# mgtools/DCTdomain

Hardware: AMD Instinct MI355X
Metric: DCT fingerprints/sec on L=500 D=1280 (higher is better)
Workload: dtype f64

## Files before the change

### dctdomain_amd/csrc/dctfp.hip

```cpp
#include "dctfp.h"

#include <hip/hip_runtime.h>

#include <dlfcn.h>
#include <execinfo.h>
#include <signal.h>
#include <unistd.h>

#include <algorithm>
#include <cmath>
#include <cstdarg>
#include <cstdio>
#include <cstring>
#include <map>
#include <mutex>
#include <new>
#include <string>
#include <unordered_map>
#include <vector>

#include "launch.h"
#include "reccut_kernel.hip.h"

using namespace dctfp;
// ... 1808 lines not shown
    return DCTFP_OK;
} DCTFP_GUARD("dctfp_scale")

int dctfp_gather_rows(dctfp_ctx* ctx, const void* embed, int32_t dtype, int64_t n_rows, int64_t n_cols, int64_t ld,
                      const dctfp_piece* pieces, int64_t n_pieces, double* out, void* stream_v) try {
    if (!ctx || !embed || !pieces || !out) return fail(DCTFP_ERR_INVALID, "dctfp_gather_rows: NULL argument");
    std::lock_guard<std::mutex> lock(ctx->mu);
    if (dtype != DCTFP_F32 && dtype != DCTFP_F64) return fail(DCTFP_ERR_INVALID, "dctfp_gather_rows: dtype %d", dtype);
    if (n_pieces < 1 || n_pieces > 65535 || n_cols < 1 || ld < n_cols) return fail(DCTFP_ERR_INVALID, "dctfp_gather_rows: bad shape");
    hipStream_t stream = (hipStream_t)stream_v;
    HIP_TRY(hipSetDevice(ctx->device));
    const size_t esz = dtype == DCTFP_F32 ? 4 : 8;
    TableLease tables(ctx->ring, stream);
    int rc = tables.stage((size_t)n_pieces * sizeof(PieceA));
    if (rc) return rc;
    PieceA* h = (PieceA*)tables.host();
    uint64_t t0 = 0;
    uint32_t max_rows = 0;
    for (int64_t i = 0; i < n_pieces; ++i) {
        const dctfp_piece& pc = pieces[i];
        if (pc.n_rows <= 0 || pc.row_start < 0 || pc.row_start + pc.n_rows > n_rows)
            return fail(DCTFP_ERR_INVALID, "dctfp_gather_rows: piece %lld outside the matrix", (long long)i);
        h[i].ptr = (const char*)embed + (size_t)pc.row_start * (size_t)ld * esz;
        h[i].n_rows = (uint32_t)pc.n_rows;
        h[i].t0 = (uint32_t)t0;
        t0 += (uint64_t)pc.n_rows;
        max_rows = std::max(max_rows, (uint32_t)pc.n_rows);
        if (t0 > 0x7fffffffu) return fail(DCTFP_ERR_LIMIT, "dctfp_gather_rows: more than 2^31 rows");
    }
    rc = tables.upload((size_t)n_pieces * sizeof(PieceA), stream);
    if (rc) return rc;
    const unsigned gx = (unsigned)std::min<int64_t>(((int64_t)max_rows * n_cols + 255) / 256, 2048);
    if (dtype == DCTFP_F32)
        hipLaunchKernelGGL((gather_rows_kernel<float>), dim3(gx, (unsigned)n_pieces), dim3(256), 0, stream, (const PieceA*)tables.dev(), (int)n_pieces, n_cols, ld, out);
    else
        hipLaunchKernelGGL((gather_rows_kernel<double>), dim3(gx, (unsigned)n_pieces), dim3(256), 0, stream, (const PieceA*)tables.dev(), (int)n_pieces, n_cols, ld, out);
    HIP_TRY(hipGetLastError());
    return tables.release();
} DCTFP_GUARD("dctfp_gather_rows")


int dctfp_contact_topk(dctfp_ctx* ctx, const void* const* maps, const int64_t* ld, const int32_t* n_res,
                       int32_t n_prot, double t, int32_t* out_i, int32_t* out_j, float* out_v,
                       const int64_t* out_offs, int32_t* out_n, void* stream_v) try {
    if (!ctx || !maps || !ld || !n_res || !out_i || !out_j || !out_v || !out_offs || !out_n)
        return fail(DCTFP_ERR_INVALID, "dctfp_contact_topk: NULL argument");
    std::lock_guard<std::mutex> lock(ctx->mu);
    if (n_prot < 0) return fail(DCTFP_ERR_INVALID, "dctfp_contact_topk: negative count");
    if (n_prot == 0) return DCTFP_OK;
    hipStream_t stream = (hipStream_t)stream_v;
    HIP_TRY(hipSetDevice(ctx->device));
    const int64_t kLongPairs = (int64_t)1 << 18;
    constexpr int64_t kStripePairs = (int64_t)1 << 17;
    auto is_long = [&](int64_t L, int64_t cand) {
        const int64_t k = dctfp_contact_count((int32_t)L, t);
        return k > 0 && (cand >= kLongPairs || (k > 3000 && cand >= ((int64_t)1 << 19)));
    };
    std::vector<int32_t> order((size_t)n_prot);
    int32_t n_short = 0, n_long = 0;
    int64_t n_stripes = 0;
    for (int32_t p = 0; p < n_prot; ++p) {
        const int64_t L = n_res[p];
        if (L < 0 || (L > 0 && (!maps[p] || ld[p] < L)))
            return fail(DCTFP_ERR_INVALID, "dctfp_contact_topk: protein %d: bad map", p);
        const int64_t cand = L >= 6 ? (L - 5) * (L - 4) / 2 : 0;
        if (is_long(L, cand)) {
            ++n_long;
            n_stripes += std::min<int64_t>(512, (cand + kStripePairs - 1) / kStripePairs);
        } else {
            ++n_short;
        }
    }
    {
        int32_t a = 0, b = n_short;
        for (int32_t p = 0; p < n_prot; ++p) {
            const int64_t L = n_res[p];
            const int64_t cand = L >= 6 ? (L - 5) * (L - 4) / 2 : 0;
            if (is_long(L, cand)) order[b++] = p;
            else order[a++] = p;
        }
    }
    const size_t off_stripe = align_up((size_t)n_prot * sizeof(TopkJob), 16);
    const size_t off_first = align_up(off_stripe + (size_t)n_stripes * sizeof(TopkStripe), 16);
    const size_t off_state = align_up(off_first + (size_t)n_long * sizeof(int32_t), 16);
    const size_t up_bytes = align_up(off_state + (size_t)n_long * sizeof(TopkState), 16);
    const size_t off_ties = up_bytes;
    const size_t all_bytes = off_ties + (size_t)n_stripes * sizeof(int32_t);
    TableLease tables(ctx->ring, stream);
    Fork fork(stream);
    int rc = tables.stage(up_bytes);
    if (rc) return rc;
    TopkJob* h = (TopkJob*)tables.host();
    TopkStripe* hs = (TopkStripe*)(tables.host() + off_stripe);
    int32_t* hfirst = (int32_t*)(tables.host() + off_first);
    TopkState* hstate = (TopkState*)(tables.host() + off_state);
    int64_t s_fill = 0;
    for (int32_t q = 0; q < n_prot; ++q) {
        const int32_t p = order[q];
        const int64_t L = n_res[p];
        h[q].map = (const float*)maps[p];
        h[q].ld = ld[p];
        h[q].n_res = (int32_t)L;
        h[q].k = (int32_t)dctfp_contact_count((int32_t)L, t);
        h[q].out_off = out_offs[p];
        h[q].orig = p;
        h[q].reserved = 0;
        if (out_offs[p + 1] - out_offs[p] < h[q].k)
            return fail(DCTFP_ERR_INVALID, "dctfp_contact_topk: protein %d: output room %lld < %d", p,
                        (long long)(out_offs[p + 1] - out_offs[p]), h[q].k);
        if (q >= n_short) {
            const int32_t lj = q - n_short;
            const int64_t cand = (L - 5) * (L - 4) / 2;
            const int64_t ns = std::min<int64_t>(512, (cand + kStripePairs - 1) / kStripePairs);
            hfirst[lj] = (int32_t)s_fill;
            memset(&hstate[lj], 0, sizeof(TopkState));
            hstate[lj].need = h[q].k;
            int64_t acc = 0;
            int32_t row = 0, stripe = 0;
            const int32_t last_row = (int32_t)L - 5;
            for (int64_t k = 0; k < ns; ++k) {
                const int64_t goal = cand * (k + 1) / ns;
                const int32_t begin = row;
                while (row < last_row && (acc < goal || k + 1 == ns)) {
                    acc += L - 5 - row;
                    ++row;
                }
                if (row > begin) {
                    TopkStripe& sp = hs[s_fill++];
                    sp.job = lj;
                    sp.row_begin = begin;
                    sp.row_end = row;
                    sp.stripe = stripe++;
                }
            }
        }
    }
    const int64_t used_stripes = s_fill;
    rc = tables.upload(up_bytes, stream, all_bytes);
    if (rc) return rc;
    const TopkJob* djobs = (const TopkJob*)tables.dev();
    const bool long_beside = n_long > 0 && used_stripes > 0 && n_short > 0;
    hipStream_t long_stream = stream;
    if (long_beside) {
        rc = ctx->ensure_cut_streams();
        if (rc == DCTFP_OK) rc = fork.fork(ctx->cut_fork);
        if (rc == DCTFP_OK) rc = fork.branch(ctx->cut[0], &long_stream);
        if (rc) return rc;
    }
    if (n_short > 0) {
        if (ctx->opt_topk_kernel != 1) {
            if (ctx->opt_topk_kernel == 0) {
                constexpr int kSmallK = 1400;
                bool any_small = false, any_large = false;
                for (int32_t q = 0; q < n_short; ++q) (h[q].k <= kSmallK ? any_small : any_large) = true;
                if (any_small)
                    hipLaunchKernelGGL((contact_topk1_kernel<8>), dim3((unsigned)n_short), dim3(512), 0, stream, djobs, out_i, out_j, out_v, out_n, 0, kSmallK);
                if (any_large)
                    hipLaunchKernelGGL((contact_topk1_kernel<16>), dim3((unsigned)n_short), dim3(1024), 0, stream, djobs, out_i, out_j, out_v, out_n,
                                       kSmallK + 1, 0x7fffffff);
            }
            hipLaunchKernelGGL(contact_topk2_kernel, dim3((unsigned)n_short), dim3(1024), 0, stream, djobs, out_i, out_j, out_v, out_n,
                               ctx->opt_topk_kernel == 0 ? 1 : 0);
            hipLaunchKernelGGL(contact_topk_kernel, dim3((unsigned)n_short), dim3(1024), 0, stream, djobs, out_i, out_j, out_v, out_n, 1);
        } else {
            hipLaunchKernelGGL(contact_topk_kernel, dim3((unsigned)n_short), dim3(1024), 0, stream, djobs, out_i, out_j, out_v, out_n, 0);
        }
        HIP_TRY(hipGetLastError());
    }
    if (n_long > 0 && used_stripes > 0) {
        stream = long_stream;
        const TopkJob* dlong = djobs + n_short;
        const TopkStripe* dstripes = (const TopkStripe*)(tables.dev() + off_stripe);
        const int32_t* dfirst = (const int32_t*)(tables.dev() + off_first);
        TopkState* dstate = (TopkState*)(tables.dev() + off_state);
        int32_t* dties = (int32_t*)(tables.dev() + off_ties);
        for (int shift = 24; shift >= 0; shift -= 8) {
            hipLaunchKernelGGL(topk_hist_kernel, dim3((unsigned)used_stripes), dim3(1024), 0, stream, dlong, dstripes, dstate, shift);
            hipLaunchKernelGGL(topk_pick_kernel, dim3((unsigned)n_long), dim3(64), 0, stream, dlong, dstate, shift, out_n);
        }
        hipLaunchKernelGGL(topk_collect_kernel, dim3((unsigned)used_stripes), dim3(1024), 0, stream, dlong, dstripes, dstate, dties, out_i,
                           out_j, out_v);
        hipLaunchKernelGGL(topk_ties_kernel, dim3((unsigned)used_stripes), dim3(64), 0, stream, dlong, dstripes, dstate, dties, dfirst,
                           out_i, out_j, out_v);
        HIP_TRY(hipGetLastError());
    }
    rc = fork.join();
    return rc ? rc : tables.release();
} DCTFP_GUARD("dctfp_contact_topk")

int dctfp_contact_sort(dctfp_ctx* ctx, const void* const* maps, const int64_t* ld, const int32_t* n_res, int32_t n_prot,
                       double t, int32_t* out_i, int32_t* out_j, float* out_v, const int64_t* out_offs, uint8_t* sorted,
                       void* stream_v) try {
    if (!ctx || !maps || !ld || !n_res || !out_i || !out_j || !out_v || !out_offs || !sorted)
        return fail(DCTFP_ERR_INVALID, "dctfp_contact_sort: NULL argument");
    std::lock_guard<std::mutex> lock(ctx->mu);
    if (n_prot < 0) return fail(DCTFP_ERR_INVALID, "dctfp_contact_sort: negative count");
    if (n_prot == 0) return DCTFP_OK;
    hipStream_t stream = (hipStream_t)stream_v;
    HIP_TRY(hipSetDevice(ctx->device));
    static const int kNet[4] = {2048, 4096, 8192, 16384};
    std::vector<int32_t> group[4];
    for (int32_t p = 0; p < n_prot; ++p) {
        const int64_t k = dctfp_contact_count(n_res[p], t);
        sorted[p] = 1;
        if (k <= 1) continue;
        if (n_res[p] > 65536 || k > kNet[3]) {
            sorted[p] = 0;
            continue;
        }
        if (!maps[p] || ld[p] < n_res[p]) return fail(DCTFP_ERR_INVALID, "dctfp_contact_sort: protein %d: bad map", p);
        int g = 0;
        while (k > kNet[g]) ++g;
        group[g].push_back(p);
    }
    const size_t n_jobs = group[0].size() + group[1].size() + group[2].size() + group[3].size();
    if (n_jobs == 0) return DCTFP_OK;
    TableLease tables(ctx->ring, stream);
    int rc = tables.stage(n_jobs * sizeof(TopkJob));
// ... 971 lines not shown
```

### dctdomain_amd/csrc/kernels.hip.h

```cpp
#pragma once

#include <hip/hip_runtime.h>
#include <stdint.h>

#include <type_traits>

namespace dctfp {

typedef double v4d __attribute__((ext_vector_type(4)));
typedef double v2d __attribute__((ext_vector_type(2)));
typedef float v4f __attribute__((ext_vector_type(4)));
typedef _Float16 v8h __attribute__((ext_vector_type(8)));
typedef _Float16 v4h __attribute__((ext_vector_type(4)));
typedef unsigned short v4us __attribute__((ext_vector_type(4)));
typedef unsigned short v8us __attribute__((ext_vector_type(8)));

typedef const double __attribute__((address_space(4))) * CosTab;
__device__ inline CosTab cos_tab(const double* p) { return (CosTab)(uintptr_t)p; }

struct bf16_t {
    unsigned short bits;
};

struct JobA {
// ... 1473 lines not shown
        bad |= (x != x) ? 1 : 0;
        mn = fmin(mn, x);
        mx = fmax(mx, x);
    }
#pragma unroll
    for (int s = 1; s < 64; s <<= 1) {
        mn = fmin(mn, __shfl_xor(mn, s));
        mx = fmax(mx, __shfl_xor(mx, s));
        bad |= __shfl_xor(bad, s);
    }
    if ((threadIdx.x & 63) == 0) {
        smn[threadIdx.x >> 6] = mn;
        smx[threadIdx.x >> 6] = mx;
        sbad[threadIdx.x >> 6] = bad;
    }
    __syncthreads();
    mn = fmin(fmin(smn[0], smn[1]), fmin(smn[2], smn[3]));
    mx = fmax(fmax(smx[0], smx[1]), fmax(smx[2], smx[3]));
    bad = sbad[0] | sbad[1] | sbad[2] | sbad[3];
    const double den = mx - mn;
    for (int64_t i = threadIdx.x; i < n; i += 256) out[i] = bad ? __builtin_nan("") : (v[i] - mn) / den;
}
#endif

template <typename T>
__global__ void gather_rows_kernel(const PieceA* __restrict__ pieces, int n_pieces, int64_t n_cols, int64_t ld,
                                   double* __restrict__ out) {
    const PieceA pc = pieces[blockIdx.y];
    const T* __restrict__ src = reinterpret_cast<const T*>(pc.ptr);
    const int64_t total = (int64_t)pc.n_rows * n_cols;
    for (int64_t i = (int64_t)blockIdx.x * blockDim.x + threadIdx.x; i < total; i += (int64_t)gridDim.x * blockDim.x) {
        const int64_t r = i / n_cols, c = i % n_cols;
        out[((int64_t)pc.t0 + r) * n_cols + c] = (double)src[r * ld + c];
    }
}


struct TopkJob {
    const float* map;
    int64_t ld;
    int32_t n_res;
    int32_t k;
    int64_t out_off;
    int32_t orig;
    int32_t reserved;
};

__device__ inline uint32_t topk_key(float v) {
    if (v == 0.0f) v = 0.0f;
    const uint32_t b = __float_as_uint(v);
    return (b & 0x80000000u) ? ~b : (b | 0x80000000u);
}

#ifndef DCTFP_TEMPLATES_ONLY
__global__ __launch_bounds__(1024) void contact_topk_kernel(const TopkJob* __restrict__ jobs,
                                                             int32_t* __restrict__ out_i, int32_t* __restrict__ out_j,
                                                             float* __restrict__ out_v, int32_t* __restrict__ out_n, int redo_only) {
    __shared__ int hist[256];
    __shared__ uint32_t s_prefix;
    __shared__ int s_need, s_eq, s_cnt;
    const TopkJob job = jobs[blockIdx.x];
    if (redo_only && out_n[job.orig] != -1) return;
    const int L = job.n_res;
    const int lane = threadIdx.x & 63, wave = threadIdx.x >> 6, nwaves = blockDim.x >> 6;
    const int last_row = L - 6;
    if (threadIdx.x == 0) {
        s_prefix = 0;
        s_need = job.k;
        s_cnt = 0;
        s_eq = 0;
    }
    __syncthreads();
    if (job.k <= 0 || last_row < 0) {
        if (threadIdx.x == 0) out_n[job.orig] = 0;
        return;
    }
    for (int shift = 24; shift >= 0; shift -= 8) {
        for (int b = threadIdx.x; b < 256; b += blockDim.x) hist[b] = 0;
        __syncthreads();
        const uint32_t prefix = s_prefix;
        for (int i = wave; i <= last_row; i += nwaves) {
            const float* __restrict__ row = job.map + (size_t)i * job.ld;
            for (int j = i + 5 + lane; j < L; j += 64) {
                const uint32_t key = topk_key(row[j]);
                if (shift == 24 || (key >> (shift + 8)) == (prefix >> (shift + 8))) atomicAdd(&hist[(key >> shift) & 255u], 1);
            }
        }
        __syncthreads();
        if (threadIdx.x == 0) {
            int need = s_need, b = 255;
            for (; b > 0; --b) {
                if (hist[b] >= need) break;
                need -= hist[b];
            }
            s_prefix = prefix | ((uint32_t)b << shift);
            s_need = need;
            s_eq = hist[b];
        }
        __syncthreads();
    }
    const uint32_t thr = s_prefix;
    const int need_eq = s_need;
    const bool all_ties = (s_eq == need_eq);
    int32_t* __restrict__ oi = out_i + job.out_off;
    int32_t* __restrict__ oj = out_j + job.out_off;
    float* __restrict__ ov = out_v + job.out_off;
    for (int i = wave; i <= last_row; i += nwaves) {
        const float* __restrict__ row = job.map + (size_t)i * job.ld;
        for (int j = i + 5 + lane; j < L; j += 64) {
            const float v = row[j];
            const uint32_t key = topk_key(v);
            if (key > thr || (all_ties && key == thr)) {
                const int pos = atomicAdd(&s_cnt, 1);
                oi[pos] = i;
                oj[pos] = j;
                ov[pos] = v;
            }
        }
    }
    __syncthreads();
    if (!all_ties && wave == 0) {
        int base = s_cnt, taken = 0;
        for (int i = 0; i <= last_row && taken < need_eq; ++i) {
            const float* __restrict__ row = job.map + (size_t)i * job.ld;
            for (int j0 = i + 5; j0 < L && taken < need_eq; j0 += 64) {
                const int j = j0 + lane;
                const float v = (j < L) ? row[j] : 0.0f;
                const bool hit = (j < L) && topk_key(v) == thr;
                const unsigned long long m = __ballot(hit);
                const int before = __popcll(m & ((1ull << lane) - 1ull));
                if (hit && taken + before < need_eq) {
                    const int pos = base + taken + before;
                    oi[pos] = i;
                    oj[pos] = j;
                    ov[pos] = v;
                }
                taken += __popcll(m);
            }
        }
    }
    if (threadIdx.x == 0) out_n[job.orig] = job.k;
}
#endif


template <int N>
__global__ __launch_bounds__(1024) void contact_sort_kernel(const TopkJob* __restrict__ jobs, int32_t* __restrict__ out_i,
                                                             int32_t* __restrict__ out_j, float* __restrict__ out_v) {
    __shared__ unsigned long long keys[N];
    const TopkJob job = jobs[blockIdx.x];
    const int k = job.k;
    if (k <= 1 || k > N) return;
    int32_t* __restrict__ oi = out_i + job.out_off;
    int32_t* __restrict__ oj = out_j + job.out_off;
    float* __restrict__ ov = out_v + job.out_off;
    for (int p = threadIdx.x; p < N; p += blockDim.x) {
        unsigned long long key = ~0ull;
        if (p < k) key = ((unsigned long long)(~topk_key(ov[p])) << 32) | ((uint32_t)oi[p] << 16) | (uint32_t)oj[p];
        keys[p] = key;
    }
    __syncthreads();
    for (int size = 2; size <= N; size <<= 1) {
        for (int stride = size >> 1; stride > 0; stride >>= 1) {
            for (int q = threadIdx.x; q < N / 2; q += blockDim.x) {
                const int lo = ((q & ~(stride - 1)) << 1) | (q & (stride - 1));
                const int hi = lo | stride;
                const bool up = (lo & size) == 0;
                const unsigned long long a = keys[lo], b = keys[hi];
                if ((a > b) == up) {
                    keys[lo] = b;
                    keys[hi] = a;
                }
            }
            __syncthreads();
        }
    }
    for (int p = threadIdx.x; p < k; p += blockDim.x) {
        const uint32_t ij = (uint32_t)keys[p];
        const int i = (int)(ij >> 16), j = (int)(ij & 0xffffu);
        oi[p] = i;
        oj[p] = j;
        ov[p] = job.map[(size_t)i * job.ld + j];
    }
}

struct TopkStripe {
    int32_t job;
    int32_t row_begin;
    int32_t row_end;
    int32_t stripe;
};

struct TopkState {
    uint32_t prefix;
// ... 701 lines not shown
        for (int i = 0; i < E; ++i) {
            const uint32_t e = (uint32_t)(i * TH + tid);
            have[i] = (e % (uint32_t)WCAP) < sh.wave_cnt[e / (uint32_t)WCAP];
            ck[i] = have[i] ? s_ckey[e] : 0xffffffffu;
            cc[i] = have[i] ? s_ccol[e] : 0xffffffffu;
        }
        bisect_emit<E>(ck, [&](int i) { return cc[i]; }, [&](int i) { return have[i]; }, row_min, bound - 1u, 0u,
                       col_hi, kk, sh, step, emit);
    } else {
        uint32_t key2[PER];
        uint32_t col2[COLS ? PER : 1];
        load_row(key2, col2);
        auto col_of2 = [&](int j) { return COLS ? col2[j] : (uint32_t)(j * TH + tid); };
        if (below < kk) bisect_emit<PER>(key2, col_of2, [&](int j) { return j < my_n; }, bound, bound, below, col_hi, kk, sh, step, emit);
        else bisect_emit<PER>(key2, col_of2, [&](int j) { return j < my_n; }, row_min, bound - 1u, 0u, col_hi, kk, sh, step, emit);
    }
    for (uint32_t pos = kk + (uint32_t)tid; pos < (uint32_t)k; pos += TH) {
        ov[pos] = 0x7fffffff;
        oi[pos] = 0x7fffffff;
    }
}


template <int N>
__global__ __launch_bounds__(N / 2) void row_order_kernel(int32_t* __restrict__ val, int32_t* __restrict__ idx, int k) {
    __shared__ unsigned long long keys[N];
    int32_t* __restrict__ v = val + (size_t)blockIdx.x * k;
    int32_t* __restrict__ c = idx + (size_t)blockIdx.x * k;
    for (int p = threadIdx.x; p < N; p += N / 2)
        keys[p] = p < k ? ((unsigned long long)((uint32_t)v[p] ^ 0x80000000u) << 32) | (uint32_t)c[p] : ~0ull;
    __syncthreads();
    for (int size = 2; size <= N; size <<= 1) {
        for (int stride = size >> 1; stride > 0; stride >>= 1) {
            const int q = threadIdx.x;
            const int lo = ((q & ~(stride - 1)) << 1) | (q & (stride - 1));
            const int hi = lo | stride;
            const bool up = (lo & size) == 0;
            const unsigned long long a = keys[lo], b = keys[hi];
            if ((a > b) == up) {
                keys[lo] = b;
                keys[hi] = a;
            }
            __syncthreads();
        }
    }
    for (int p = threadIdx.x; p < k; p += N / 2) {
        v[p] = (int32_t)((uint32_t)(keys[p] >> 32) ^ 0x80000000u);
        c[p] = (int32_t)(uint32_t)keys[p];
    }
}

constexpr int kTopkCap = 8192;
template <int M>
__device__ inline void topk2_run(const TopkJob& job, SelectShared& sh, uint32_t* __restrict__ s_key, uint32_t* __restrict__ s_ij,
                                 int32_t* __restrict__ out_i, int32_t* __restrict__ out_j, float* __restrict__ out_v,
                                 int32_t* __restrict__ out_n) {
    const int L = job.n_res, last_row = L - 6;
    const int tid = threadIdx.x, lane = tid & 63, wave = tid >> 6;
    const uint32_t kk = (uint32_t)job.k;
    auto ikey = [](float v) { return ~topk_key(v); };
    const __amdgpu_buffer_rsrc_t mb = __builtin_amdgcn_make_buffer_rsrc(const_cast<float*>(job.map), 0, (int)((int64_t)L * job.ld * 4), 0x00020000);
    auto stream = [&](auto f) {
        constexpr int G = 12;
        const int n_rows = last_row >= wave ? (last_row - wave) / 16 + 1 : 0;
        for (int n = 0; 2 * n < n_rows; ++n) {
            const int ra = wave + 16 * n, rb = wave + 16 * (n_rows - 1 - n);
            const int ca = (L - 5 - ra + 63) >> 6, cb = rb != ra ? (L - 5 - rb + 63) >> 6 : 0;
            const int la = (lane + ra * 13) & 63, lb = (lane + rb * 13) & 63;
            for (int s0 = 0; s0 < ca + cb; s0 += G) {
                float v[G];
#pragma unroll
                for (int u = 0; u < G; ++u) {
                    const int sl = s0 + u;
                    const int i = sl < ca ? ra : rb, c = sl < ca ? sl : sl - ca;
                    v[u] = __builtin_bit_cast(float, __builtin_amdgcn_raw_buffer_load_b32(mb, (sl < ca ? la : lb) * 4,
                                                                                          (int)(((int64_t)i * job.ld + i + 5 + 64 * c) * 4), 0));
                }
#pragma unroll
                for (int u = 0; u < G; ++u) {
                    const int sl = s0 + u;
                    const int i = sl < ca ? ra : rb, c = sl < ca ? sl : sl - ca;
                    const int j = i + 5 + 64 * c + (sl < ca ? la : lb);
                    f(i, j, v[u], sl < ca + cb && j < L);
                }
            }
        }
    };
    uint32_t t[M];
#pragma unroll
    for (int m = 0; m < M; ++m) t[m] = 0xffffffffu;
    stream([&](int, int, float v, bool valid) {
        uint32_t x = valid ? ikey(v) : 0xffffffffu;
#pragma unroll
        for (int m = 0; m < M; ++m) {
            const uint32_t lo = min(t[m], x);
            x = max(t[m], x);
            t[m] = lo;
        }
    });
    int step = 0;
    uint32_t n_less = 0;
    const uint32_t bound = kth_smallest<M>(t, 0u, 0xffffffffu, n_less, kk, sh, step);
    stream([&](int i, int j, float v, bool valid) {
        const uint32_t x = ikey(v);
        const bool take = valid && x <= bound;
        const unsigned long long mask = __builtin_amdgcn_ballot_w64(take);
        if (mask != 0) {
            uint32_t base = 0;
            if (lane == 0) base = atomicAdd(&sh.fill, (uint32_t)__builtin_popcountll(mask));
            base = (uint32_t)__builtin_amdgcn_readfirstlane((int)base);
            const uint32_t at = base + __builtin_amdgcn_mbcnt_hi((uint32_t)(mask >> 32), __builtin_amdgcn_mbcnt_lo((uint32_t)mask, 0u));
            if (take && at < (uint32_t)kTopkCap) {
                s_key[at] = x;
                s_ij[at] = ((uint32_t)i << 16) | (uint32_t)j;
            }
        }
    });
    __syncthreads();
    const uint32_t n_cand = sh.fill;
    if (n_cand > (uint32_t)kTopkCap) {
        if (tid == 0) out_n[job.orig] = -1;
        return;
    }
    constexpr int E = kTopkCap / 1024;
    uint32_t ck[E], cij[E];
#pragma unroll
    for (int e = 0; e < E; ++e) {
        const uint32_t p = (uint32_t)(e * 1024 + tid);
        ck[e] = p < n_cand ? s_key[p] : 0xffffffffu;
        cij[e] = p < n_cand ? s_ij[p] : 0xffffffffu;
    }
    int32_t* __restrict__ oi = out_i + job.out_off;
    int32_t* __restrict__ oj = out_j + job.out_off;
    float* __restrict__ ov = out_v + job.out_off;
    bisect_emit<E>(ck, [&](int e) { return cij[e]; }, [&](int e) { return (uint32_t)(e * 1024 + tid) < n_cand; }, 0u, bound, 0u, 0xfffffffeu, kk, sh,
                   step, [&](uint32_t pos, uint32_t, uint32_t ij) {
                       const int i = (int)(ij >> 16), j = (int)(ij & 0xffffu);
                       oi[pos] = i;
                       oj[pos] = j;
                       ov[pos] = job.map[(size_t)i * job.ld + j];
                   });
    if (tid == 0) out_n[job.orig] = job.k;
}

#ifndef DCTFP_TOPK_WAVES
#define DCTFP_TOPK_WAVES 8
#endif
#ifndef DCTFP_TEMPLATES_ONLY
__global__ __launch_bounds__(1024, DCTFP_TOPK_WAVES) void contact_topk2_kernel(const TopkJob* __restrict__ jobs, int32_t* __restrict__ out_i,
                                                              int32_t* __restrict__ out_j, float* __restrict__ out_v,
                                                              int32_t* __restrict__ out_n, int redo_only) {
    __shared__ SelectShared sh;
    __shared__ uint32_t s_key[kTopkCap], s_ij[kTopkCap];
    const TopkJob job = jobs[blockIdx.x];
    if (redo_only && out_n[job.orig] >= 0) return;
    if (threadIdx.x < kSelectCounters) sh.cnt[threadIdx.x] = 0;
    if (threadIdx.x == 0) {
        sh.pos = 0;
        sh.fill = 0;
    }
    __syncthreads();
    if (job.k <= 0 || job.n_res < 6) {
        if (threadIdx.x == 0) out_n[job.orig] = 0;
        return;
    }
    if (job.k > 6144 || job.n_res > 65535 || (int64_t)job.n_res * job.ld >= ((int64_t)1 << 29)) {
        if (threadIdx.x == 0) out_n[job.orig] = -1;
        return;
    }
    if (job.k <= 1400) topk2_run<2>(job, sh, s_key, s_ij, out_i, out_j, out_v, out_n);
    else if (job.k <= 3000) topk2_run<4>(job, sh, s_key, s_ij, out_i, out_j, out_v, out_n);
    else topk2_run<8>(job, sh, s_key, s_ij, out_i, out_j, out_v, out_n);
}
#endif

template <bool VEC4, int NW>
struct TopkSlots {
    static constexpr int W = VEC4 ? 4 : 1, CH = 64 * W;
    int L, wave, n_rows, n_pairs;
    int n, sl, ra, rb, ca, cb;
    __device__ inline static int first_col(int i) { return VEC4 ? ((i + 5) & ~3) : i + 5; }
    __device__ inline int chunks(int i) const { return (L - first_col(i) + CH - 1) / CH; }
    __device__ inline void set_pair(int pair) {
        n = pair;
        sl = 0;
        if (pair < n_pairs) {
            ra = wave + NW * pair;
            rb = wave + NW * (n_rows - 1 - pair);
            ca = chunks(ra);
            cb = rb != ra ? chunks(rb) : 0;
        } else {
            ra = rb = 0;
            ca = cb = 0;
        }
    }
    __device__ inline void init(int L_, int wave_) {
        L = L_;
        wave = wave_;
        const int last_row = L - 6;
        n_rows = last_row >= wave ? (last_row - wave) / NW + 1 : 0;
        n_pairs = (n_rows + 1) / 2;
        set_pair(0);
    }
    __device__ inline bool done() const { return n >= n_pairs; }
    __device__ inline int row() const { return sl < ca ? ra : rb; }
    __device__ inline int col0() const { return first_col(row()) + CH * (sl < ca ? sl : sl - ca); }
    __device__ inline void next() {
        if (++sl >= ca + cb) set_pair(n + 1);
    }
};

template <bool VEC4, int NW>
__device__ inline void topk1_run(const TopkJob& job, SelectSharedT<NW>& sh, uint32_t* __restrict__ s_key, uint32_t* __restrict__ s_ij,
                                 uint16_t* __restrict__ s_rowt, uint32_t* __restrict__ s_rowp, int32_t* __restrict__ out_i,
                                 int32_t* __restrict__ out_j, float* __restrict__ out_v, int32_t* __restrict__ out_n) {
    constexpr int kRowTies = NW == 8 ? 576 : 1216;
    constexpr int W = VEC4 ? 4 : 1, NS = 4;
    constexpr int WCAP = 512;
    constexpr int TH = NW * 64;
    typedef typename std::conditional<VEC4, v4f, float>::type LV;
    const int L = job.n_res;
    const int tid = threadIdx.x, lane = tid & 63, wave = __builtin_amdgcn_readfirstlane(tid >> 6);
    const uint32_t kk = (uint32_t)job.k;
    auto ikey = [](float v) { return ~topk_key(v); };
    auto load = [&](int i, int c0) -> LV {
        const __amdgpu_buffer_rsrc_t rb = __builtin_amdgcn_make_buffer_rsrc(const_cast<float*>(job.map) + (int64_t)max(i, 0) * job.ld, 0,
                                                                               i >= 0 ? L * 4 : 0, 0x00020000);
        if constexpr (VEC4) return __builtin_bit_cast(v4f, __builtin_amdgcn_raw_buffer_load_b128(rb, lane * 16, c0 * 4, 0));
        else return __builtin_bit_cast(float, __builtin_amdgcn_raw_buffer_load_b32(rb, lane * 4, c0 * 4, 0));
    };
    auto elem = [](const LV& v, int e) -> float {
        if constexpr (VEC4) return v[e];
        else return v;
    };
    TopkSlots<VEC4, NW> it;
    it.init(L, wave);
    const int stride = it.n_pairs >= NS ? it.n_pairs / NS : 1;
    int s_row[NS], s_c0[NS], s_pair[NS], s_slot[NS];
    LV sv[NS];
#pragma unroll
    for (int u = 0; u < NS; ++u) {
        TopkSlots<VEC4, NW> p = it;
        p.set_pair(u * stride);
        s_pair[u] = s_slot[u] = -1;
        s_row[u] = -1;
        s_c0[u] = 0;
        if (!p.done()) {
            const int want = (u + 1) % (p.ca + p.cb);
            for (int q = 0; q < want; ++q) p.next();
            s_pair[u] = p.n;
            s_slot[u] = p.sl;
            s_row[u] = p.row();
            s_c0[u] = p.col0();
        }
    }
#pragma unroll
    for (int u = 0; u < NS; ++u) sv[u] = load(s_row[u], s_c0[u]);
    uint32_t sk[NS * W];
    uint32_t n_w = 0, s_valid = 0;
    uint32_t kmin = 0xffffffffu, kmax = 0;
#pragma unroll
    for (int u = 0; u < NS; ++u)
#pragma unroll
        for (int e = 0; e < W; ++e) {
            const int j = s_c0[u] + W * lane + e;
            const bool valid = s_pair[u] >= 0 && j >= s_row[u] + 5 && j < L;
            const uint32_t x = ikey(elem(sv[u], e));
            sk[u * W + e] = valid ? x : 0xffffffffu;
// ... 77 lines not shown
    };
#pragma unroll
    for (int u = 0; u < NS; ++u)
#pragma unroll
        for (int e = 0; e < W; ++e) offer(elem(sv[u], e), [&]() { return (bool)((s_valid >> (u * W + e)) & 1u); }, max(s_row[u], 0), s_c0[u] + W * lane + e);
    constexpr int G = VEC4 ? 8 : 12;
    if (!whole) {
        auto sampled = [&](const TopkSlots<VEC4, NW>& p) {
            bool hit = false;
#pragma unroll
            for (int u = 0; u < NS; ++u) hit |= p.n == s_pair[u] && p.sl == s_slot[u];
            return hit;
        };
        while (!it.done()) {
            LV v[G];
            int vi[G], vc[G];
#pragma unroll
            for (int u = 0; u < G; ++u) {
                while (!it.done() && sampled(it)) it.next();
                vi[u] = -1;
                vc[u] = 0;
                if (!it.done()) {
                    vi[u] = it.row();
                    vc[u] = it.col0();
                    it.next();
                }
            }
#pragma unroll
            for (int u = 0; u < G; ++u) v[u] = load(vi[u], vc[u]);
#pragma unroll
            for (int u = 0; u < G; ++u) {
                if (vi[u] < 0) continue;
#pragma unroll
                for (int e = 0; e < W; ++e) {
                    const int j = vc[u] + W * lane + e;
                    offer(elem(v[u], e), [&]() { return j >= vi[u] + 5 && j < L; }, vi[u], j);
                }
            }
        }
    }
    if (lane == 0) sh.wave_cnt[wave] = w_fill;
    __syncthreads();
    uint32_t n_cand = 0;
    bool over = false;
    for (int w = 0; w < NW; ++w) {
        n_cand += sh.wave_cnt[w];
        over |= sh.wave_cnt[w] > (uint32_t)WCAP;
    }
#if defined(DCTFP_TOPK1_STOP) && DCTFP_TOPK1_STOP == 2
    if (tid == 0) out_n[job.orig] = (int)n_cand;
    return;
#endif
    if (over || (!count_ties && n_cand < kk)) {
        if (tid == 0) out_n[job.orig] = -1;
        return;
    }
    constexpr int E = WCAP / 64;
    uint32_t ck[E], cij[E];
    bool have[E];
    uint32_t cmin = 0xffffffffu;
    const uint32_t key_hi = count_ties ? (bound == 0 ? 0u : bound - 1u) : bound;
#pragma unroll
    for (int e = 0; e < E; ++e) {
        const uint32_t p = (uint32_t)(e * TH + tid);
        have[e] = (p % (uint32_t)WCAP) < sh.wave_cnt[p / (uint32_t)WCAP];
        const uint32_t xk = have[e] ? ikey(__uint_as_float(s_key[p])) : 0xffffffffu;
        have[e] = have[e] && xk <= key_hi && (!count_ties || bound != 0);
        ck[e] = have[e] ? xk : 0xffffffffu;
        cij[e] = have[e] ? s_ij[p] : 0xffffffffu;
        cmin = min(cmin, ck[e]);
    }
#pragma unroll
    for (int off = 32; off >= 1; off >>= 1) cmin = min(cmin, (uint32_t)__shfl_xor((int)cmin, off));
    uint32_t n_real = 0;
#pragma unroll
    for (int e = 0; e < E; ++e) n_real += lane_votes(have[e]);
    if (lane == 0) {
        atomicMin(&sh.row_min, cmin);
        atomicAdd(&sh.fill, n_real);
    }
    __syncthreads();
    cmin = sh.row_min;
    const uint32_t n_less = sh.fill;
    int32_t* __restrict__ oi = out_i + job.out_off;
    int32_t* __restrict__ oj = out_j + job.out_off;
    float* __restrict__ ov = out_v + job.out_off;
    auto emit = [&](uint32_t pos, uint32_t key_e, uint32_t ij) {
        const int i = (int)(ij >> 16), j = (int)(ij & 0xffffu);
        oi[pos] = i;
        oj[pos] = j;
        const uint32_t tk = ~key_e;
        const float val = __uint_as_float((tk & 0x80000000u) ? (tk & 0x7fffffffu) : ~tk);
        ov[pos] = val == 0.0f ? job.map[(size_t)i * job.ld + j] : val;
    };
    if (n_less >= kk) {
        bisect_emit<E>(ck, [&](int e) { return cij[e]; }, [&](int e) { return have[e]; }, cmin, key_hi, 0u, 0xfffffffeu, kk, sh, step, emit);
        if (tid == 0) out_n[job.orig] = job.k;
        return;
    }
    if (!count_ties) {
        if (tid == 0) out_n[job.orig] = -1;
        return;
    }
    const uint32_t need = kk - n_less;
    if (wave == 0) {
        uint32_t carry = 0;
        for (int r0 = 0; r0 < L; r0 += 64) {
            const int r = r0 + lane;
            const uint32_t c = r < L ? s_rowt[r] : 0u;
            uint32_t incl = c;
#pragma unroll
            for (int off = 1; off < 64; off <<= 1) {
                const uint32_t up = (uint32_t)__shfl_up((int)incl, off);
                incl += lane >= off ? up : 0u;
            }
            if (r < L) s_rowp[r] = carry + incl - c;
            carry += (uint32_t)__builtin_amdgcn_readlane((int)incl, 63);
        }
        if (lane == 0) sh.bound = carry;
    }
    __syncthreads();
    if (sh.bound < need) {
        if (tid == 0) out_n[job.orig] = -1;
        return;
    }
#pragma unroll
    for (int e = 0; e < E; ++e) {
        const unsigned long long mask = __builtin_amdgcn_ballot_w64(have[e]);
        if (mask != 0) {
            uint32_t base = 0;
            if (lane == 0) base = atomicAdd(&sh.pos, (uint32_t)__builtin_popcountll(mask));
            base = (uint32_t)__builtin_amdgcn_readfirstlane((int)base);
            if (have[e]) emit(base + __builtin_amdgcn_mbcnt_hi((uint32_t)(mask >> 32), __builtin_amdgcn_mbcnt_lo((uint32_t)mask, 0u)), ck[e], cij[e]);
        }
    }
    {
        TopkSlots<VEC4, NW> it2;
        it2.init(L, wave);
        int cur_row = -1;
        uint32_t row_run = 0;
        while (!it2.done()) {
            LV v[G];
            int vi[G], vc[G];
#pragma unroll
            for (int u = 0; u < G; ++u) {
                while (!it2.done() && s_rowp[it2.row()] >= need) it2.next();
                vi[u] = -1;
                vc[u] = 0;
                if (!it2.done()) {
                    vi[u] = it2.row();
                    vc[u] = it2.col0();
                    it2.next();
                }
            }
#pragma unroll
            for (int u = 0; u < G; ++u) v[u] = load(vi[u], vc[u]);
#pragma unroll
            for (int u = 0; u < G; ++u) {
                if (vi[u] < 0) continue;
                if (vi[u] != cur_row) {
                    cur_row = vi[u];
                    row_run = 0;
                }
                unsigned long long m[W];
                uint32_t total = 0;
#pragma unroll
                for (int e = 0; e < W; ++e) {
                    const int j = vc[u] + W * lane + e;
                    m[e] = __builtin_amdgcn_ballot_w64(j >= vi[u] + 5 && j < L && elem(v[u], e) == thr);
                    total += (uint32_t)__builtin_popcountll(m[e]);
                }
                if (total == 0) continue;
                const unsigned long long lower = (1ull << lane) - 1ull;
                uint32_t before_lane = 0;
#pragma unroll
                for (int e = 0; e < W; ++e) before_lane += (uint32_t)__builtin_popcountll(m[e] & lower);
                uint32_t mine = 0;
#pragma unroll
                for (int e = 0; e < W; ++e) {
                    if ((m[e] >> lane) & 1ull) {
                        const uint32_t at = s_rowp[vi[u]] + row_run + before_lane + mine;
                        if (at < need) {
                            const int j = vc[u] + W * lane + e;
                            oi[n_less + at] = vi[u];
                            oj[n_less + at] = j;
                            ov[n_less + at] = elem(v[u], e);
                        }
                        ++mine;
                    }
                }
                row_run += total;
            }
        }
    }
    if (tid == 0) out_n[job.orig] = job.k;
}

template <int NW>
__global__ __launch_bounds__(NW * 64, DCTFP_TOPK_WAVES) void contact_topk1_kernel(const TopkJob* __restrict__ jobs, int32_t* __restrict__ out_i,
                                                              int32_t* __restrict__ out_j, float* __restrict__ out_v,
                                                              int32_t* __restrict__ out_n, int k_from, int k_to) {
    __shared__ SelectSharedT<NW> sh;
    __shared__ uint32_t s_key[NW * 512], s_ij[NW * 512];
    __shared__ uint16_t s_rowt[NW == 8 ? 576 : 1216];
    const TopkJob job = jobs[blockIdx.x];
    if (job.k > 0 && job.n_res >= 6 && (job.k < k_from || job.k > k_to)) return;
    for (int q = threadIdx.x; q < kSelectCounters; q += NW * 64) sh.cnt[q] = 0;
    if (threadIdx.x == 0) {
        sh.pos = 0;
        sh.fill = 0;
        sh.row_min = 0xffffffffu;
    }
    __syncthreads();
    if (job.k <= 0 || job.n_res < 6) {
        if (threadIdx.x == 0) out_n[job.orig] = 0;
        return;
    }
    if (job.k > 3000 || job.n_res > 65535 || (int64_t)job.n_res * job.ld >= ((int64_t)1 << 29)) {
        if (threadIdx.x == 0) out_n[job.orig] = -1;
        return;
    }
    if ((reinterpret_cast<uintptr_t>(job.map) & 15u) == 0 && (job.ld & 3) == 0) topk1_run<true, NW>(job, sh, s_key, s_ij, s_rowt, s_ij, out_i, out_j, out_v, out_n);
    else topk1_run<false, NW>(job, sh, s_key, s_ij, s_rowt, s_ij, out_i, out_j, out_v, out_n);
}

}
```

Baseline: 1.370 million.

## Group short top-k jobs by k and run fallback kernels only over a redo list

Short contact-topk jobs are now sorted on the host into k-size groups, so each topk1 variant launches only over its own group instead of the full job count with early-exit blocks. Jobs that cannot finish in a fast path append their index to a device-side redo list via an atomic counter. The topk2 and generic fallback kernels then walk only that list with a capped, grid-strided launch instead of spawning one block per job that mostly exits. This cuts empty block launches, at the cost of an extra atomic per failed job, a device-read loop bound, and slightly more staging memory.

```diff
diff --git a/dctdomain_amd/csrc/dctfp.hip b/dctdomain_amd/csrc/dctfp.hip
--- a/dctdomain_amd/csrc/dctfp.hip
+++ b/dctdomain_amd/csrc/dctfp.hip
@@ -1884,40 +1884,45 @@
     HIP_TRY(hipSetDevice(ctx->device));
     const int64_t kLongPairs = (int64_t)1 << 18;
     constexpr int64_t kStripePairs = (int64_t)1 << 17;
-    auto is_long = [&](int64_t L, int64_t cand) {
-        const int64_t k = dctfp_contact_count((int32_t)L, t);
-        return k > 0 && (cand >= kLongPairs || (k > 3000 && cand >= ((int64_t)1 << 19)));
-    };
-    std::vector<int32_t> order((size_t)n_prot);
-    int32_t n_short = 0, n_long = 0;
+    constexpr int kBuilds = 2;
+    static const int32_t kBuildK[kBuilds] = {1400, 0x7fffffff};
+    std::vector<int32_t> order((size_t)n_prot), k_of((size_t)n_prot);
+    std::vector<uint8_t> group((size_t)n_prot);
+    int32_t n_group[kBuilds + 1] = {};
     int64_t n_stripes = 0;
     for (int32_t p = 0; p < n_prot; ++p) {
         const int64_t L = n_res[p];
         if (L < 0 || (L > 0 && (!maps[p] || ld[p] < L)))
             return fail(DCTFP_ERR_INVALID, "dctfp_contact_topk: protein %d: bad map", p);
         const int64_t cand = L >= 6 ? (L - 5) * (L - 4) / 2 : 0;
-        if (is_long(L, cand)) {
-            ++n_long;
+        const int64_t k = dctfp_contact_count((int32_t)L, t);
+        k_of[p] = (int32_t)k;
+        int g = 0;
+        if (k > 0 && (cand >= kLongPairs || (k > 3000 && cand >= ((int64_t)1 << 19)))) {
+            g = kBuilds;
             n_stripes += std::min<int64_t>(512, (cand + kStripePairs - 1) / kStripePairs);
         } else {
-            ++n_short;
-        }
-    }
+            while (k > kBuildK[g]) ++g;
+        }
+        group[p] = (uint8_t)g;
+        ++n_group[g];
+    }
+    int32_t first[kBuilds + 2] = {};
+    for (int g = 0; g <= kBuilds; ++g) first[g + 1] = first[g] + n_group[g];
+    const int32_t n_short = first[kBuilds], n_long = n_group[kBuilds];
     {
-        int32_t a = 0, b = n_short;
-        for (int32_t p = 0; p < n_prot; ++p) {
-            const int64_t L = n_res[p];
-            const int64_t cand = L >= 6 ? (L - 5) * (L - 4) / 2 : 0;
-            if (is_long(L, cand)) order[b++] = p;
-            else order[a++] = p;
-        }
+        int32_t at[kBuilds + 1];
+        std::copy(first, first + kBuilds + 1, at);
+        for (int32_t p = 0; p < n_prot; ++p) order[at[group[p]]++] = p;
     }
     const size_t off_stripe = align_up((size_t)n_prot * sizeof(TopkJob), 16);
     const size_t off_first = align_up(off_stripe + (size_t)n_stripes * sizeof(TopkStripe), 16);
     const size_t off_state = align_up(off_first + (size_t)n_long * sizeof(int32_t), 16);
-    const size_t up_bytes = align_up(off_state + (size_t)n_long * sizeof(TopkState), 16);
+    const size_t off_redo_n = align_up(off_state + (size_t)n_long * sizeof(TopkState), 16);
+    const size_t up_bytes = off_redo_n + 16;
     const size_t off_ties = up_bytes;
-    const size_t all_bytes = off_ties + (size_t)n_stripes * sizeof(int32_t);
+    const size_t off_redo = align_up(off_ties + (size_t)n_stripes * sizeof(int32_t), 16);
+    const size_t all_bytes = off_redo + 2 * (size_t)n_short * sizeof(int32_t);
     TableLease tables(ctx->ring, stream);
     Fork fork(stream);
     int rc = tables.stage(up_bytes);
@@ -1926,6 +1931,7 @@
     TopkStripe* hs = (TopkStripe*)(tables.host() + off_stripe);
     int32_t* hfirst = (int32_t*)(tables.host() + off_first);
     TopkState* hstate = (TopkState*)(tables.host() + off_state);
+    memset(tables.host() + off_redo_n, 0, 16);
     int64_t s_fill = 0;
     for (int32_t q = 0; q < n_prot; ++q) {
         const int32_t p = order[q];
@@ -1933,7 +1939,7 @@
         h[q].map = (const float*)maps[p];
         h[q].ld = ld[p];
         h[q].n_res = (int32_t)L;
-        h[q].k = (int32_t)dctfp_contact_count((int32_t)L, t);
+        h[q].k = k_of[p];
         h[q].out_off = out_offs[p];
         h[q].orig = p;
         h[q].reserved = 0;
@@ -1980,22 +1986,29 @@
         if (rc) return rc;
     }
     if (n_short > 0) {
+        uint32_t* redo_n = (uint32_t*)(tables.dev() + off_redo_n);
+        int32_t* redo1 = (int32_t*)(tables.dev() + off_redo);
+        int32_t* redo2 = redo1 + n_short;
+        const unsigned redo_grid = (unsigned)std::min<int32_t>(n_short, 512);
         if (ctx->opt_topk_kernel != 1) {
             if (ctx->opt_topk_kernel == 0) {
-                constexpr int kSmallK = 1400;
-                bool any_small = false, any_large = false;
-                for (int32_t q = 0; q < n_short; ++q) (h[q].k <= kSmallK ? any_small : any_large) = true;
-                if (any_small)
-                    hipLaunchKernelGGL((contact_topk1_kernel<8>), dim3((unsigned)n_short), dim3(512), 0, stream, djobs, out_i, out_j, out_v, out_n, 0, kSmallK);
-                if (any_large)
-                    hipLaunchKernelGGL((contact_topk1_kernel<16>), dim3((unsigned)n_short), dim3(1024), 0, stream, djobs, out_i, out_j, out_v, out_n,
-                                       kSmallK + 1, 0x7fffffff);
+                if (n_group[0] > 0)
+                    hipLaunchKernelGGL((contact_topk1_kernel<8>), dim3((unsigned)n_group[0]), dim3(512), 0, stream, djobs, first[0], out_i, out_j,
+                                       out_v, out_n, 0, kBuildK[0], redo_n, redo1);
+                if (n_group[1] > 0)
+                    hipLaunchKernelGGL((contact_topk1_kernel<16>), dim3((unsigned)n_group[1]), dim3(1024), 0, stream, djobs, first[1], out_i, out_j,
+                                       out_v, out_n, kBuildK[0] + 1, kBuildK[1], redo_n, redo1);
+                hipLaunchKernelGGL(contact_topk2_kernel, dim3(redo_grid), dim3(1024), 0, stream, djobs, out_i, out_j, out_v, out_n,
+                                   (const uint32_t*)redo_n, (const int32_t*)redo1, redo_n + 1, redo2);
+            } else {
+                hipLaunchKernelGGL(contact_topk2_kernel, dim3((unsigned)n_short), dim3(1024), 0, stream, djobs, out_i, out_j, out_v, out_n,
+                                   (const uint32_t*)nullptr, (const int32_t*)nullptr, redo_n + 1, redo2);
             }
-            hipLaunchKernelGGL(contact_topk2_kernel, dim3((unsigned)n_short), dim3(1024), 0, stream, djobs, out_i, out_j, out_v, out_n,
-                               ctx->opt_topk_kernel == 0 ? 1 : 0);
-            hipLaunchKernelGGL(contact_topk_kernel, dim3((unsigned)n_short), dim3(1024), 0, stream, djobs, out_i, out_j, out_v, out_n, 1);
+            hipLaunchKernelGGL(contact_topk_kernel, dim3(redo_grid), dim3(1024), 0, stream, djobs, out_i, out_j, out_v, out_n,
+                               (const uint32_t*)(redo_n + 1), (const int32_t*)redo2);
         } else {
-            hipLaunchKernelGGL(contact_topk_kernel, dim3((unsigned)n_short), dim3(1024), 0, stream, djobs, out_i, out_j, out_v, out_n, 0);
+            hipLaunchKernelGGL(contact_topk_kernel, dim3((unsigned)n_short), dim3(1024), 0, stream, djobs, out_i, out_j, out_v, out_n,
+                               (const uint32_t*)nullptr, (const int32_t*)nullptr);
         }
         HIP_TRY(hipGetLastError());
     }
diff --git a/dctdomain_amd/csrc/kernels.hip.h b/dctdomain_amd/csrc/kernels.hip.h
--- a/dctdomain_amd/csrc/kernels.hip.h
+++ b/dctdomain_amd/csrc/kernels.hip.h
@@ -1549,15 +1549,18 @@
     return (b & 0x80000000u) ? ~b : (b | 0x80000000u);
 }
 
+__device__ inline void topk_hand_back(const TopkJob& job, int q, int32_t* __restrict__ out_n, uint32_t* __restrict__ redo_n,
+                                      int32_t* __restrict__ redo) {
+    out_n[job.orig] = -1;
+    redo[atomicAdd(redo_n, 1u)] = q;
+}
+
 #ifndef DCTFP_TEMPLATES_ONLY
-__global__ __launch_bounds__(1024) void contact_topk_kernel(const TopkJob* __restrict__ jobs,
-                                                             int32_t* __restrict__ out_i, int32_t* __restrict__ out_j,
-                                                             float* __restrict__ out_v, int32_t* __restrict__ out_n, int redo_only) {
+__device__ inline void contact_topk_job(const TopkJob& job, int32_t* __restrict__ out_i, int32_t* __restrict__ out_j,
+                                        float* __restrict__ out_v, int32_t* __restrict__ out_n) {
     __shared__ int hist[256];
     __shared__ uint32_t s_prefix;
     __shared__ int s_need, s_eq, s_cnt;
-    const TopkJob job = jobs[blockIdx.x];
-    if (redo_only && out_n[job.orig] != -1) return;
     const int L = job.n_res;
     const int lane = threadIdx.x & 63, wave = threadIdx.x >> 6, nwaves = blockDim.x >> 6;
     const int last_row = L - 6;
@@ -1637,6 +1640,23 @@
         }
     }
     if (threadIdx.x == 0) out_n[job.orig] = job.k;
+}
+
+__global__ __launch_bounds__(1024) void contact_topk_kernel(const TopkJob* __restrict__ jobs,
+                                                             int32_t* __restrict__ out_i, int32_t* __restrict__ out_j,
+                                                             float* __restrict__ out_v, int32_t* __restrict__ out_n,
+                                                             const uint32_t* __restrict__ todo_n, const int32_t* __restrict__ todo) {
+    if (!todo_n) {
+        const TopkJob job = jobs[blockIdx.x];
+        contact_topk_job(job, out_i, out_j, out_v, out_n);
+        return;
+    }
+    const uint32_t n = *todo_n;
+    for (uint32_t q = blockIdx.x; q < n; q += gridDim.x) {
+        const TopkJob job = jobs[todo[q]];
+        contact_topk_job(job, out_i, out_j, out_v, out_n);
+        __syncthreads();
+    }
 }
 #endif
 
@@ -2444,9 +2464,9 @@
 
 constexpr int kTopkCap = 8192;
 template <int M>
-__device__ inline void topk2_run(const TopkJob& job, SelectShared& sh, uint32_t* __restrict__ s_key, uint32_t* __restrict__ s_ij,
+__device__ inline void topk2_run(const TopkJob& job, int q, SelectShared& sh, uint32_t* __restrict__ s_key, uint32_t* __restrict__ s_ij,
                                  int32_t* __restrict__ out_i, int32_t* __restrict__ out_j, float* __restrict__ out_v,
-                                 int32_t* __restrict__ out_n) {
+                                 int32_t* __restrict__ out_n, uint32_t* __restrict__ redo_n, int32_t* __restrict__ redo) {
     const int L = job.n_res, last_row = L - 6;
     const int tid = threadIdx.x, lane = tid & 63, wave = tid >> 6;
     const uint32_t kk = (uint32_t)job.k;
@@ -2511,7 +2531,7 @@
     __syncthreads();
     const uint32_t n_cand = sh.fill;
     if (n_cand > (uint32_t)kTopkCap) {
-        if (tid == 0) out_n[job.orig] = -1;
+        if (tid == 0) topk_hand_back(job, q, out_n, redo_n, redo);
         return;
     }
     constexpr int E = kTopkCap / 1024;
@@ -2539,13 +2559,9 @@
 #define DCTFP_TOPK_WAVES 8
 #endif
 #ifndef DCTFP_TEMPLATES_ONLY
-__global__ __launch_bounds__(1024, DCTFP_TOPK_WAVES) void contact_topk2_kernel(const TopkJob* __restrict__ jobs, int32_t* __restrict__ out_i,
-                                                              int32_t* __restrict__ out_j, float* __restrict__ out_v,
-                                                              int32_t* __restrict__ out_n, int redo_only) {
-    __shared__ SelectShared sh;
-    __shared__ uint32_t s_key[kTopkCap], s_ij[kTopkCap];
-    const TopkJob job = jobs[blockIdx.x];
-    if (redo_only && out_n[job.orig] >= 0) return;
+__device__ inline void contact_topk2_job(const TopkJob& job, int q, SelectShared& sh, uint32_t* __restrict__ s_key, uint32_t* __restrict__ s_ij,
+                                         int32_t* __restrict__ out_i, int32_t* __restrict__ out_j, float* __restrict__ out_v,
+                                         int32_t* __restrict__ out_n, uint32_t* __restrict__ redo_n, int32_t* __restrict__ redo) {
     if (threadIdx.x < kSelectCounters) sh.cnt[threadIdx.x] = 0;
     if (threadIdx.x == 0) {
         sh.pos = 0;
@@ -2557,12 +2573,33 @@
         return;
     }
     if (job.k > 6144 || job.n_res > 65535 || (int64_t)job.n_res * job.ld >= ((int64_t)1 << 29)) {
-        if (threadIdx.x == 0) out_n[job.orig] = -1;
+        if (threadIdx.x == 0) topk_hand_back(job, q, out_n, redo_n, redo);
         return;
     }
-    if (job.k <= 1400) topk2_run<2>(job, sh, s_key, s_ij, out_i, out_j, out_v, out_n);
-    else if (job.k <= 3000) topk2_run<4>(job, sh, s_key, s_ij, out_i, out_j, out_v, out_n);
-    else topk2_run<8>(job, sh, s_key, s_ij, out_i, out_j, out_v, out_n);
+    if (job.k <= 1400) topk2_run<2>(job, q, sh, s_key, s_ij, out_i, out_j, out_v, out_n, redo_n, redo);
+    else if (job.k <= 3000) topk2_run<4>(job, q, sh, s_key, s_ij, out_i, out_j, out_v, out_n, redo_n, redo);
+    else topk2_run<8>(job, q, sh, s_key, s_ij, out_i, out_j, out_v, out_n, redo_n, redo);
+}
+
+__global__ __launch_bounds__(1024, DCTFP_TOPK_WAVES) void contact_topk2_kernel(const TopkJob* __restrict__ jobs, int32_t* __restrict__ out_i,
+                                                              int32_t* __restrict__ out_j, float* __restrict__ out_v,
+                                                              int32_t* __restrict__ out_n, const uint32_t* __restrict__ todo_n,
+                                                              const int32_t* __restrict__ todo, uint32_t* __restrict__ redo_n,
+                                                              int32_t* __restrict__ redo) {
+    __shared__ SelectShared sh;
+    __shared__ uint32_t s_key[kTopkCap], s_ij[kTopkCap];
+    if (!todo_n) {
+        const TopkJob job = jobs[blockIdx.x];
+        contact_topk2_job(job, (int)blockIdx.x, sh, s_key, s_ij, out_i, out_j, out_v, out_n, redo_n, redo);
+        return;
+    }
+    const uint32_t n = *todo_n;
+    for (uint32_t at = blockIdx.x; at < n; at += gridDim.x) {
+        const int q = todo[at];
+        const TopkJob job = jobs[q];
+        contact_topk2_job(job, q, sh, s_key, s_ij, out_i, out_j, out_v, out_n, redo_n, redo);
+        __syncthreads();
+    }
 }
 #endif
 
@@ -2603,9 +2640,10 @@
 };
 
 template <bool VEC4, int NW>
-__device__ inline void topk1_run(const TopkJob& job, SelectSharedT<NW>& sh, uint32_t* __restrict__ s_key, uint32_t* __restrict__ s_ij,
+__device__ inline void topk1_run(const TopkJob& job, int q, SelectSharedT<NW>& sh, uint32_t* __restrict__ s_key, uint32_t* __restrict__ s_ij,
                                  uint16_t* __restrict__ s_rowt, uint32_t* __restrict__ s_rowp, int32_t* __restrict__ out_i,
-                                 int32_t* __restrict__ out_j, float* __restrict__ out_v, int32_t* __restrict__ out_n) {
+                                 int32_t* __restrict__ out_j, float* __restrict__ out_v, int32_t* __restrict__ out_n,
+                                 uint32_t* __restrict__ redo_n, int32_t* __restrict__ redo) {
     constexpr int kRowTies = NW == 8 ? 576 : 1216;
     constexpr int W = VEC4 ? 4 : 1, NS = 4;
     constexpr int WCAP = 512;
@@ -2789,7 +2827,7 @@
     return;
 #endif
     if (over || (!count_ties && n_cand < kk)) {
-        if (tid == 0) out_n[job.orig] = -1;
+        if (tid == 0) topk_hand_back(job, q, out_n, redo_n, redo);
         return;
     }
     constexpr int E = WCAP / 64;
@@ -2836,7 +2874,7 @@
         return;
     }
     if (!count_ties) {
-        if (tid == 0) out_n[job.orig] = -1;
+        if (tid == 0) topk_hand_back(job, q, out_n, redo_n, redo);
         return;
     }
     const uint32_t need = kk - n_less;
@@ -2858,7 +2896,7 @@
     }
     __syncthreads();
     if (sh.bound < need) {
-        if (tid == 0) out_n[job.orig] = -1;
+        if (tid == 0) topk_hand_back(job, q, out_n, redo_n, redo);
         return;
     }
 #pragma unroll
@@ -2934,15 +2972,17 @@
 }
 
 template <int NW>
-__global__ __launch_bounds__(NW * 64, DCTFP_TOPK_WAVES) void contact_topk1_kernel(const TopkJob* __restrict__ jobs, int32_t* __restrict__ out_i,
+__global__ __launch_bounds__(NW * 64, DCTFP_TOPK_WAVES) void contact_topk1_kernel(const TopkJob* __restrict__ jobs, int first, int32_t* __restrict__ out_i,
                                                               int32_t* __restrict__ out_j, float* __restrict__ out_v,
-                                                              int32_t* __restrict__ out_n, int k_from, int k_to) {
+                                                              int32_t* __restrict__ out_n, int k_from, int k_to,
+                                                              uint32_t* __restrict__ redo_n, int32_t* __restrict__ redo) {
     __shared__ SelectSharedT<NW> sh;
     __shared__ uint32_t s_key[NW * 512], s_ij[NW * 512];
     __shared__ uint16_t s_rowt[NW == 8 ? 576 : 1216];
-    const TopkJob job = jobs[blockIdx.x];
+    const int q = first + (int)blockIdx.x;
+    const TopkJob job = jobs[q];
     if (job.k > 0 && job.n_res >= 6 && (job.k < k_from || job.k > k_to)) return;
-    for (int q = threadIdx.x; q < kSelectCounters; q += NW * 64) sh.cnt[q] = 0;
+    for (int c = threadIdx.x; c < kSelectCounters; c += NW * 64) sh.cnt[c] = 0;
     if (threadIdx.x == 0) {
         sh.pos = 0;
         sh.fill = 0;
@@ -2954,11 +2994,11 @@
         return;
     }
     if (job.k > 3000 || job.n_res > 65535 || (int64_t)job.n_res * job.ld >= ((int64_t)1 << 29)) {
-        if (threadIdx.x == 0) out_n[job.orig] = -1;
+        if (threadIdx.x == 0) topk_hand_back(job, q, out_n, redo_n, redo);
         return;
     }
-    if ((reinterpret_cast<uintptr_t>(job.map) & 15u) == 0 && (job.ld & 3) == 0) topk1_run<true, NW>(job, sh, s_key, s_ij, s_rowt, s_ij, out_i, out_j, out_v, out_n);
-    else topk1_run<false, NW>(job, sh, s_key, s_ij, s_rowt, s_ij, out_i, out_j, out_v, out_n);
-}
-
-}
+    if ((reinterpret_cast<uintptr_t>(job.map) & 15u) == 0 && (job.ld & 3) == 0) topk1_run<true, NW>(job, q, sh, s_key, s_ij, s_rowt, s_ij, out_i, out_j, out_v, out_n, redo_n, redo);
+    else topk1_run<false, NW>(job, q, sh, s_key, s_ij, s_rowt, s_ij, out_i, out_j, out_v, out_n, redo_n, redo);
+}
+
+}
```

After: 1.369 million. No clear change (-0.0%).
